# ubisoft/ubisoft-laforge-msmd

Measured on AMD Instinct MI355X. Metric: FLAME frames/sec on 4s@16kHz clips (whole job; MSMD.forward motion-coefficient frames), higher is better.
Workload: dtype bf16; 1 GPU; configs[1]: MSMD.forward, batch=32 x 4 s clips per GPU, wav2vec2-base encoder + 8-layer motion decoder, eval-mode, synthetic closed-form weights; batch_per_gpu=32, frames_per_clip=100, parallelism=dp1 (independent clips, no collective), launch=one hipGraph replay per step (the batch sits in the captured input buffers)

## Files before the change

include/msmd_hip.h:

```cpp
#ifndef MSMD_HIP_H
#define MSMD_HIP_H

#include <stdint.h>

#ifdef __cplusplus
extern "C" {
#endif

#define MSMD_F32 0
#define MSMD_BF16 1
#define MSMD_F16 2
#define MSMD_F16X2 3

#define MSMD_ACT_NONE 0
#define MSMD_ACT_GELU 1
#define MSMD_ACT_ELU 2

typedef void* msmd_stream_t;

int msmd_abi_version(void);
#define MSMD_GEMM_VARIANT(v) ((v) << 8)
#define MSMD_GEMM_WRITE_THROUGH (1 << 16)
#define MSMD_GEMM_PAIRED_STORES (1 << 17)
#define MSMD_GEMM_STAGGER (1 << 18)
// ... 21 lines not shown
                 long ldr, int act, int batch, long strideA, long strideW, long strideC, long strideBias, long strideR,
                 void* z_out, float p_drop, const unsigned long* rng_state, unsigned int site, msmd_stream_t stream);

int msmd_gemm_route(const void* A, const void* W, const float* bias, const void* residual, void* C, int M, int N, int K,
                    int in_dtype, int out_dtype, long lda, int rows_per_batch, long a_batch_stride, long ldw, long ldc,
                    long ldr, int act, int batch, long strideA, long strideW, long strideC, long strideBias, long strideR,
                    void* z_out, float p_drop, const unsigned long* rng_state, unsigned int site, msmd_stream_t stream);
int msmd_gemm_ln_route(const void* A, const void* W, const float* bias, const void* residual, void* C, int M, int N, int K,
                       int in_dtype, int out_dtype, long lda, long ldw, long ldc, long ldr, int act, const float* a_stats,
                       const float* w_colsum, const float* r_stats, const float* r_gamma, const float* r_beta,
                       float* stats_out, int slab_in, int slab_out, float eps, msmd_stream_t stream);
int msmd_gemm_ln_rows(const void* A, const void* W, const float* bias, const void* residual, void* C, int M, int N, int K,
                      int in_dtype, int out_dtype, long lda, long ldw, long ldc, long ldr, int act, const float* a_stats,
                      const float* w_colsum, const float* r_stats, const float* r_gamma, const float* r_beta,
                      float* stats_out, int slab_in, int slab_out, float eps, msmd_stream_t stream);

int msmd_gemm_actbwd(const void* A, const void* W, const void* Z, void* C, int M, int N, int K, int in_dtype, int out_dtype,
                     long lda, long ldw, int act, float p_drop, const unsigned long* rng_state, unsigned int site,
                     msmd_stream_t stream);

int msmd_gemm_batched2(const void* A, const void* W, void* C, int M, int N, int K, int in_dtype, int out_dtype,
                       long lda, long ldw, long ldc, int batch_outer, long strideA_o, long strideW_o, long strideC_o,
                       int batch_inner, long strideA_i, long strideW_i, long strideC_i, msmd_stream_t stream);

int msmd_gemm_tn(const void* A, const void* B, float* C, float* colsum, int M, int N, int K, long lda, long ldb,
                 long ldc, int batch, long strideA, long strideB, long strideC, int b_rows_per_window,
                 long b_window_stride, int accumulate, void* ws, long ws_bytes, msmd_stream_t stream);
long msmd_gemm_tn_workspace(int M, int N, int K, int batch);

int msmd_layernorm(const void* x, const void* residual, const float* gamma, const float* beta,
// ... 361 lines not shown
```

ubisoft-laforge-msmd_amd/csrc/gemm.hip:

```cpp
#include "gemm_tiles.h"
#include <atomic>
#include <utility>

struct GemmArgs {
  const void* A; const void* W; const float* bias; const void* R; void* C;
  int M, N, K;
  long lda; int rows_per_batch; long a_batch_stride; long ldw, ldc, ldr;
  int act; int vec_ok; float inv_rpb;
  long strideA, strideW, strideC, strideBias, strideR;
  int mt, nt;
  int batch_inner; long strideA2, strideW2, strideC2;
  void* Z; float p_drop; const unsigned long* rng; unsigned site;
  int xn;
  int flags;
  const float* a_stats = nullptr; int a_nt = 0; const float* w_colsum = nullptr;
  const float* r_stats = nullptr; int r_nt = 0; const float* r_gamma = nullptr; const float* r_beta = nullptr;
  float* stats_out = nullptr; float ln_eps = 1e-5f;
  int stagger_ticks = 0;
};

enum : int {
  GF_WRITE_THROUGH = 1, GF_PAIRED_STORES = 2, GF_STAGGER = 4,
  GF_ACT_BWD = 8,
  GF_ONE_TILE = 16, GF_NO_256 = 32,
// ... 905 lines not shown
        }
    }
    stage = ring_next<NSTAGE>(stage);
  }
#pragma unroll
  for (int i = 0; i < FN; ++i)
#pragma unroll
    for (int j = 0; j < FM; ++j)
#pragma unroll
      for (int e = 0; e < 4; ++e)
        acc0[i][j][e] = WS ? acc0[i][j][e] * MSMD_SPLIT_INV : fmaf(acc1[i][j][e], MSMD_SPLIT_INV, acc0[i][j][e]);
  if constexpr (sizeof(TO) == 4) gemm_epilogue<float, FM, FN, false, false, ACTK>(p, acc0, z, m0 + wm, n0 + wn, fr, fq);
  else gemm_epilogue_split<FM, FN, ACTK>(p, acc0, z, m0 + wm, n0 + wn, fr, fq);
}

template <typename TI, int EPIA, int SPLIT = 0>
__global__ __launch_bounds__(512) __attribute__((amdgpu_waves_per_eu(2, 2))) void gemm8_kernel(const GemmArgs p) {
  typedef typename std::conditional<(SPLIT & 3) == 2, float, TI>::type TO;
  constexpr bool WS = (SPLIT & 4) != 0;
  constexpr int EPI = epia_family(EPIA), ACTK = epia_act(EPIA);
  static_assert(SPLIT == 0 || (EPI == 1 && __is_same(TI, f16_t)), "split operands: fp16 planes, plain epilogue");
  constexpr int HALF = 128 * 128;
  constexpr int BUF = 4 * HALF;
  extern __shared__ __attribute__((aligned(16))) unsigned char smem[];

  const int pid = blockIdx.x, ntiles = p.mt * p.nt, nwg = gridDim.x;
  const int xcd = pid & 7;
  const int run0 = (xcd < (ntiles & 7) ? xcd * ((ntiles >> 3) + 1) : (ntiles & 7) * ((ntiles >> 3) + 1) + (xcd - (ntiles & 7)) * (ntiles >> 3));
  const int run_n = (ntiles >> 3) + (xcd < (ntiles & 7) ? 1 : 0);
  const int stride = (nwg >> 3) + (xcd < (nwg & 7) ? 1 : 0);
  int tl = pid >> 3;
  const bf16_t* __restrict__ A = (const bf16_t*)p.A;
  const bf16_t* __restrict__ W = (const bf16_t*)p.W;
  const int tid = threadIdx.x, lane = tid & 63;
  const int wid = __builtin_amdgcn_readfirstlane(tid >> 6);
  const int wr = wid >> 2, wc = wid & 3;

  unsigned src[4][2];
  int m0 = 0, n0 = 0;
  auto set_tile = [&](int t) {
    const int m_tile = (run0 + t) / p.nt, n_tile = (run0 + t) - m_tile * p.nt;
    m0 = m_tile * 256; n0 = n_tile * 256;
    int ln = lane;
    asm volatile("" : "+v"(ln));
#pragma unroll
    for (int i = 0; i < 2; ++i) {
      const int row = (i * 8 + wid) * 8 + (ln >> 3), phys = ln & 7;
      const int c = phys ^ ((row >> 1) & 7);
#pragma unroll
      for (int h = 0; h < 2; ++h) {
        src[h][i] = (unsigned)((a_row_offset(p, min(m0 + h * 128 + row, p.M - 1)) + c * 8) * 2);
        src[2 + h][i] = (unsigned)(((long)min(n0 + h * 128 + row, p.N - 1) * p.ldw + c * 8) * 2);
      }
    }
  };
  const unsigned dma_base = wid * 1024;
  auto stage = [&](int which, int kt, unsigned bufoff) {
// ... 105 lines not shown
        int ll = lane;
        asm volatile("" : "+v"(ll));
        const int m = min(m0 + ((ll >> 2) & 3) * 64 + wid * 8 + (ll & 3) * 2, p.M - 2);
#pragma unroll
        for (int q = 0; q < 4; ++q) {
          if (4 * q < ln_nt) {
            const int t = min(4 * q + (ll >> 4), ln_nt - 1);
            __builtin_amdgcn_global_load_lds((gbl_void_t*)(ln_stats + ((long)t * p.M + m) * 2),
                                             (lds_void_t*)(smem + (2 * BUF + wid * 4096 + q * 1024)), 16, 0, 0);
          }
        }
      }
    }
  };

  const int nk = p.K / (SPLIT ? 32 : 64);
  typedef typename Vec4T<TO>::type V4;
  const bool has_r = p.R != nullptr;
  const bool wt = p.flags & GF_WRITE_THROUGH;

  set_tile(tl);
  ln_request();
  stage(2, 0, 0); stage(0, 0, 0); stage(3, 0, 0); stage(1, 0, 0);
  stage(2, 1, BUF); stage(0, 1, BUF); stage(3, 1, BUF);
  asm volatile("s_waitcnt vmcnt(6)" ::: "memory");
  __builtin_amdgcn_s_barrier();

  while (true) {
    if (wr == 1) __builtin_amdgcn_s_barrier();
#pragma unroll
    for (int h = 0; h < 2; ++h)
#pragma unroll
      for (int g = 0; g < 2; ++g)
#pragma unroll
        for (int i = 0; i < 2; ++i)
#pragma unroll
          for (int j = 0; j < 4; ++j) acc[h][g][i][j] = f32x4{0.f, 0.f, 0.f, 0.f};
    unsigned cur = 0;
    auto ktile = [&](int t, auto MODE_) {
      constexpr int MODE = decltype(MODE_)::value;
      read_w(0, fw0);
      __builtin_amdgcn_sched_barrier(0);
      read_x(0);
      if (MODE <= 1) stage(1, t + 1, cur ^ BUF);
      asm volatile("s_waitcnt lgkmcnt(8)" ::: "memory");
      if constexpr (WS) scale_w(fw0, fs0);
      G8_BAR();
      quadrant(acc[0][0], fw0, fs0);
      G8_BAR();
      read_w(1, fw1);
      if (MODE == 0) stage(2, t + 2, cur);
      if constexpr (WS) {
        asm volatile("s_waitcnt lgkmcnt(0)" ::: "memory");
        scale_w(fw1, fs1);
      }
      G8_BAR();
      quadrant(acc[0][1], fw1, fs1);
      G8_BAR();
      read_x(1);
      if (MODE == 0) stage(0, t + 2, cur);
      G8_BAR();
      quadrant(acc[1][1], fw1, fs1);
      G8_BAR();
      if (MODE == 0) stage(3, t + 2, cur);
      if (MODE == 0) asm volatile("s_waitcnt vmcnt(6)" ::: "memory");
      if (MODE == 1) asm volatile("s_waitcnt vmcnt(0)" ::: "memory");
      G8_BAR();
      quadrant(acc[1][0], fw0, fs0);
      G8_BAR();
      cur ^= BUF; xa0 ^= BUF; xa1 ^= BUF; wa0 ^= BUF; wa1 ^= BUF;
    };
    for (int t = 0; t < nk - 2; ++t) ktile(t, std::integral_constant<int, 0>{});
    ktile(nk - 2, std::integral_constant<int, 1>{});
    ktile(nk - 1, std::integral_constant<int, 2>{});
    if (wr == 0) __builtin_amdgcn_s_barrier();
    if (nk & 1) { xa0 ^= BUF; xa1 ^= BUF; wa0 ^= BUF; wa1 ^= BUF; }

    const int em0 = m0, en0 = n0;
    int el = lane;
    asm volatile("" : "+v"(el));
    const int efr = el & 15, efq = el >> 4;
    const int ncol = en0 + el * 4;
    f32x4 cbias = f32x4{0.f, 0.f, 0.f, 0.f}, cx = f32x4{1.f, 1.f, 1.f, 1.f}, cy = f32x4{0.f, 0.f, 0.f, 0.f};
    if (p.bias) cbias = *(const f32x4*)(p.bias + ncol);
    if constexpr (EPI == 2) cx = *(const f32x4*)(p.w_colsum + ncol);
    if constexpr (EPI == 3) {
      if (p.r_stats) { cx = *(const f32x4*)(p.r_gamma + ncol); cy = *(const f32x4*)(p.r_beta + ncol); }
    }
    float mu_l = 0.f, rs_l = 1.f;
    if constexpr (EPI >= 2) {
      if (ln_stats) {
        const int r32 = el & 31;
        const unsigned base = 2 * BUF + wid * 4096 + (((r32 >> 3) * 4 + ((r32 & 7) >> 1)) << 4) + ((r32 & 1) << 3);
        float Sf[4], Qf[4];
#pragma unroll
        for (int f = 0; f < 4; ++f) {
          f32x2 w[4];
#pragma unroll
          for (int q = 0; q < 4; ++q) {
// ... 5 lines not shown
          Qf[f] = (w[0][1] + w[1][1]) + (w[2][1] + w[3][1]);
        }
        if (ln_nt > 16) {
          const f32x2* rp = (const f32x2*)ln_stats + min(em0 + (r32 >> 3) * 64 + wid * 8 + (r32 & 7), p.M - 1);
#pragma unroll
          for (int f = 0; f < 4; ++f)
            for (int t = 16 + f; t < ln_nt; t += 4) { const f32x2 w = rp[(long)t * p.M]; Sf[f] += w[0]; Qf[f] += w[1]; }
        }
        const float S = (Sf[0] + Sf[1]) + (Sf[2] + Sf[3]), Q = (Qf[0] + Qf[1]) + (Qf[2] + Qf[3]);
        const float inv_cols = 1.0f / (float)(EPI == 2 ? p.K : p.N);
        mu_l = S * inv_cols;
        rs_l = rsqrtf(fmaxf(Q * inv_cols - mu_l * mu_l, 0.f) + p.ln_eps);
        asm volatile("s_waitcnt lgkmcnt(0)" ::: "memory");
      }
    }
    tl += stride;
    const bool more = tl < run_n;
    if (more) {
      set_tile(tl);
      stage(2, 0, 0); stage(0, 0, 0); stage(3, 0, 0); stage(1, 0, 0);
      ln_request();
    }
    auto write_block = [&](const f32x4 (&q0)[2][4], const f32x4 (&q1)[2][4]) {
#pragma unroll
      for (int g = 0; g < 2; ++g)
#pragma unroll
        for (int i = 0; i < 2; ++i)
#pragma unroll
          for (int j = 0; j < 4; ++j) {
            const int row = j * 16 + efr, c = g * 32 + wc * 8 + i * 4 + efq;
            *(f32x4*)(smem + BUF + row * 1024 + ((c ^ efr) << 4)) = g == 0 ? q0[i][j] : q1[i][j];
          }
    };
    auto finish_block = [&](int ps) {
      if constexpr ((SPLIT & 3) == 2) {
        f32x4 rr[8];
        if (has_r) {
#pragma unroll
          for (int it = 0; it < 8; ++it) {
            const int m = min(em0 + ps * 64 + wid * 8 + it, p.M - 1);
            rr[it] = *(const f32x4*)((const float*)p.R + (long)m * p.ldr + ncol);
          }
        }
#pragma unroll
        for (int it = 0; it < 8; ++it) {
          const int row = wid * 8 + it, m = em0 + ps * 64 + row;
          const f32x4 a = *(const f32x4*)(smem + BUF + row * 1024 + ((el ^ (row & 15)) << 4));
          f32x4 o;
#pragma unroll
          for (int e = 0; e < 4; ++e) {
            o[e] = act_out_c<float, ACTK>(WS ? fmaf(a[e], MSMD_SPLIT_INV, cbias[e]) : a[e] + cbias[e], p.act);
            if (has_r) o[e] += rr[it][e];
          }
          if (m < p.M) {
            if (wt) store16_wt((float*)p.C + (long)m * p.ldc + ncol, __builtin_bit_cast(u32x4, o));
            else *(f32x4*)((float*)p.C + (long)m * p.ldc + ncol) = o;
          }
        }
      } else if constexpr ((SPLIT & 3) == 1) {
        const bool odd = el & 1;
        const long coff = 2L * en0 + ((el >> 3) << 6) + (((el >> 1) & 3) << 3) + (odd ? 32 : 0);
        auto swap1 = [](unsigned x) { return (unsigned)__builtin_amdgcn_mov_dpp((int)x, 0xB1, 0xF, 0xF, false); };
        u32x4 rr[8];
        if (has_r) {
#pragma unroll
          for (int it = 0; it < 8; ++it) {
            const int m = min(em0 + ps * 64 + wid * 8 + it, p.M - 1);
            rr[it] = *(const u32x4*)((const f16_t*)p.R + (long)m * 2 * p.ldr + coff);
          }
        }
#pragma unroll
        for (int it = 0; it < 8; ++it) {
          const int row = wid * 8 + it, m = em0 + ps * 64 + row;
          const f32x4 a = *(const f32x4*)(smem + BUF + row * 1024 + ((el ^ (row & 15)) << 4));
          float v[4];
#pragma unroll
          for (int e = 0; e < 4; ++e) v[e] = act_split<ACTK>(WS ? fmaf(a[e], MSMD_SPLIT_INV, cbias[e]) : a[e] + cbias[e], p.act);
          if (has_r) {
            const unsigned g0 = swap1(odd ? rr[it][0] : rr[it][2]), g1 = swap1(odd ? rr[it][1] : rr[it][3]);
            const f16x2 h01 = __builtin_bit_cast(f16x2, odd ? g0 : rr[it][0]), h23 = __builtin_bit_cast(f16x2, odd ? g1 : rr[it][1]);
            const f16x2 l01 = __builtin_bit_cast(f16x2, odd ? rr[it][2] : g0), l23 = __builtin_bit_cast(f16x2, odd ? rr[it][3] : g1);
            v[0] += unsplit_f16x2(h01[0], l01[0]); v[1] += unsplit_f16x2(h01[1], l01[1]);
            v[2] += unsplit_f16x2(h23[0], l23[0]); v[3] += unsplit_f16x2(h23[1], l23[1]);
          }
          f16_t h[4], l[4];
#pragma unroll
          for (int e = 0; e < 4; ++e) split_f16x2(v[e], h[e], l[e]);
          const unsigned hp0 = __builtin_bit_cast(unsigned, f16x2{h[0], h[1]}), hp1 = __builtin_bit_cast(unsigned, f16x2{h[2], h[3]});
          const unsigned lp0 = __builtin_bit_cast(unsigned, f16x2{l[0], l[1]}), lp1 = __builtin_bit_cast(unsigned, f16x2{l[2], l[3]});
          const unsigned g0 = swap1(odd ? hp0 : lp0), g1 = swap1(odd ? hp1 : lp1);
          const u32x4 o = odd ? u32x4{g0, g1, lp0, lp1} : u32x4{hp0, hp1, g0, g1};
          if (m < p.M) {
            if (wt) store16_wt((f16_t*)p.C + (long)m * 2 * p.ldc + coff, o);
            else *(u32x4*)((f16_t*)p.C + (long)m * 2 * p.ldc + coff) = o;
          }
        }
      } else {
      V4 rr[8];
      if (EPI != 2 && has_r) {
#pragma unroll
        for (int it = 0; it < 8; ++it) {
          const int m = min(em0 + ps * 64 + wid * 8 + it, p.M - 1);
          rr[it] = *(const V4*)((const TO*)p.R + (long)m * p.ldr + ncol);
        }
      }
#pragma unroll
      for (int it = 0; it < 8; ++it) {
        const int row = wid * 8 + it, m = em0 + ps * 64 + row;
        const f32x4 a = *(const f32x4*)(smem + BUF + row * 1024 + ((el ^ (row & 15)) << 4));
        float mu = 0.f, rs = 1.f;
        if constexpr (EPI >= 2) {
          mu = __int_as_float(__builtin_amdgcn_readlane(__float_as_int(mu_l), ps * 8 + it));
          rs = __int_as_float(__builtin_amdgcn_readlane(__float_as_int(rs_l), ps * 8 + it));
        }
        float v[4];
#pragma unroll
        for (int e = 0; e < 4; ++e) {
          float x = a[e];
          if constexpr (EPI == 2) x = rs * (x - mu * cx[e]);
          v[e] = act_out_c<TO, ACTK>(x + cbias[e], p.act);
          if constexpr (EPI == 3) v[e] += fmaf(((float)rr[it][e] - mu) * rs, cx[e], cy[e]);
          else if (has_r) v[e] += (float)rr[it][e];
        }
        const V4 o = pack4<TO>(v[0], v[1], v[2], v[3]);
        if (m < p.M) {
          if (wt) store8_wt((TO*)p.C + (long)m * p.ldc + ncol, __builtin_bit_cast(u32x2, o));
          else *(V4*)((TO*)p.C + (long)m * p.ldc + ncol) = o;
        }
        if constexpr (EPI == 3) {
          if (p.stats_out) {
            float S = 0.f, Q = 0.f;
#pragma unroll
            for (int e = 0; e < 4; ++e) { const float w = (float)o[e]; S += w; Q = fmaf(w, w, Q); }
#pragma unroll
            for (int d : {4, 8, 1, 2}) { S += __shfl_xor(S, d, 64); Q += __shfl_xor(Q, d, 64); }
            if ((el & 15) == 0 && m < p.M) *(f32x2*)(p.stats_out + ((long)((en0 >> 6) + (el >> 4)) * p.M + m) * 2) = f32x2{S, Q};
          }
        }
      }
      }
    };
    if (wr == 0) write_block(acc[0][0], acc[0][1]);
    G8_EBAR();
    finish_block(0);
    G8_EBAR();
    if (wr == 1) write_block(acc[0][0], acc[0][1]);
    G8_EBAR();
    finish_block(1);
    G8_EBAR();
    if (wr == 0) write_block(acc[1][0], acc[1][1]);
    G8_EBAR();
    finish_block(2);
    G8_EBAR();
    if (wr == 1) write_block(acc[1][0], acc[1][1]);
    G8_EBAR();
    finish_block(3);
    if (!more) break;
    G8_EBAR();
    set_tile(tl);
    stage(2, 1, BUF); stage(0, 1, BUF); stage(3, 1, BUF);
    asm volatile("s_waitcnt vmcnt(6)" ::: "memory");
    __builtin_amdgcn_s_barrier();
  }
#undef G8_BAR
#undef G8_EBAR
}

template <int... CODES, typename F>
static int dispatch_code(int code, F&& f) {
  int r = -1;
  (void)((code == CODES && ((r = f(std::integral_constant<int, CODES>{})), true)) || ...);
  return r;
}

template <auto KFN>
static int gemm_launch_kernel(dim3 grid, int threads, int lds, hipStream_t st, const GemmArgs& p) {
  if (lds > 0) {
    static std::atomic<unsigned long> allowed{0};
    int dev = 0;
    (void)hipGetDevice(&dev);
    const unsigned long bit = (unsigned)dev < 64 ? 1UL << dev : 0;
    if (!(allowed.load(std::memory_order_relaxed) & bit)) {
      (void)hipFuncSetAttribute((const void*)KFN, hipFuncAttributeMaxDynamicSharedMemorySize, lds);
      allowed.fetch_or(bit, std::memory_order_relaxed);
    }
  }
  hipLaunchKernelGGL(KFN, grid, dim3(threads), lds, st, p);
  MSMD_RETURN_LAST();
}

static int gemm2_xcd_grid(GemmArgs& p, int BM, int BN, long lda) {
  p.mt = (p.M + BM - 1) / BM; p.nt = (p.N + BN - 1) / BN;
  const double a_bytes = 2.0 * p.M * (double)(p.rows_per_batch < p.M ? lda : p.K), w_bytes = 2.0 * p.N * (double)p.K;
  double best = 1e30;
  int want_xn = 1;
  for (int xn = 1; xn <= 4; xn *= 2) {
    const double c = 0.7 * xn * a_bytes + (8.0 / xn) * w_bytes;
    if (c < best && p.nt >= xn) { best = c; want_xn = xn; }
  }
  p.xn = p.nt >= want_xn ? want_xn : 1;
  const int xm_n = 8 / p.xn;
  return ((p.mt + xm_n - 1) / xm_n) * ((p.nt + p.xn - 1) / p.xn) * 8;
// ... 433 lines not shown
  c.lda = lda; c.ldw = ldw; c.ldc = N; c.act = act & (0xffff | MSMD_GEMM_WRITE_THROUGH | MSMD_GEMM_PAIRED_STORES);
  c.z_out = const_cast<void*>(Z); c.p_drop = p_drop; c.rng = rng_state; c.site = site; c.internal_flags = GF_ACT_BWD;
  return gemm_run(gemm_plan, c, stream);
}

extern "C" int msmd_gemm_batched2(const void* A, const void* W, void* C, int M, int N, int K, int in_dtype, int out_dtype, long lda, long ldw,
                                  long ldc, int batch_outer, long strideA_o, long strideW_o, long strideC_o, int batch_inner, long strideA_i,
                                  long strideW_i, long strideC_i, msmd_stream_t stream) {
  GemmCall c;
  c.A = A; c.W = W; c.C = C; c.M = M; c.N = N; c.K = K; c.in_dtype = in_dtype; c.out_dtype = out_dtype;
  c.lda = lda; c.ldw = ldw; c.ldc = ldc; c.act = MSMD_ACT_NONE;
  c.batch = batch_outer; c.strideA = strideA_o; c.strideW = strideW_o; c.strideC = strideC_o;
  c.batch_inner = batch_inner; c.strideA2 = strideA_i; c.strideW2 = strideW_i; c.strideC2 = strideC_i;
  return gemm_run(gemm_plan, c, stream);
}
```

ubisoft-laforge-msmd_amd/ops.py:

```python
from __future__ import annotations

import ctypes
import functools
import os

import numpy as np
import torch
from torch.autograd.function import once_differentiable

from . import _lib

_HEADER = _lib.parse_constants()


def _h(*names):
    vals = tuple(_HEADER["MSMD_" + n] for n in names)
    return vals if len(vals) > 1 else vals[0]


F32, BF16, F16, F16X2 = _h("F32", "BF16", "F16", "F16X2")
SPLIT = "f16x2"


class Split:
# ... 382 lines not shown
    _lib.check(lib.msmd_gemm_tn(_p(a), _p(b), _p(out), _p(cs), M, N, K, lda, ldb, K, batch, strideA, strideB, N * K,
                                b_rows_per_window, b_window_stride, int(bool(accumulate)) | (int(splits) << 8), _p(ws), nws,
                                _stream()), "msmd_gemm_tn")
    return (out, cs) if (want_colsum or colsum_out is not None) else out


def conv1d_cl(x, w_packed, bias=None, *, kernel, stride, act=ACT_NONE, out_dtype=None):
    B, T, C = x.shape
    T_out = (T - kernel) // stride + 1
    out = empty((B, T_out, w_packed.shape[0]), x.device, out_dtype or x.dtype)
    gemm(x, w_packed, bias, None, act, out=out, M=B * T_out, K=kernel * C, lda=stride * C, rows_per_batch=T_out,
         a_batch_stride=T * C)
    return out


def layernorm(x, gamma, beta, residual=None, post_add=None, act=ACT_NONE, eps=1e-5, out_dtype=None, post_act=ACT_NONE,
              split=None):
    _need_cuda(x, gamma, beta)
    lib = _lib.load()
    cols = x.shape[-1]
    rows = x.numel() // cols
    if split:
        if x.dtype != torch.float32 or (residual is not None and residual.dtype != torch.float32):
            raise TypeError("layernorm(split=...) takes fp32 input")
        y = torch.empty(x.shape, device=x.device, dtype=torch.float32) if split == "both" else None
        ys = empty(tuple(x.shape), x.device, SPLIT)
        _lib.check(lib.msmd_layernorm_f16x2(_p(x), _p(residual), _p(gamma), _p(beta), _p(post_add), _p(y), _p(ys), rows,
                                            cols, eps, act | (post_act << 8), _stream()), "msmd_layernorm_f16x2")
        return (y, ys) if split == "both" else ys
    y = torch.empty(x.shape, device=x.device, dtype=out_dtype or x.dtype)
# ... 1367 lines not shown
```

ubisoft-laforge-msmd_amd/train_graph.py:

```python
from __future__ import annotations

import os
from types import SimpleNamespace

import numpy as np
import torch

from . import autograd as ag
from . import ops
from .utils.model_common import pad_audio_plan
from .utils.wav2vec2 import compute_mask_indices, compute_mask_indices_hf


USE_CONV3_FN = os.environ.get("MSMD_CONV3_FN", "1") != "0"


def _p(tree, name):
    return tree.get(name) if hasattr(tree, "get") else getattr(tree, name)


class PosConvFn(torch.autograd.Function):

    @staticmethod
    def forward(ctx, h, w, bias):
# ... 188 lines not shown
    if noise.graph_safe:
        coins = torch.rand((groups, 1, 1) if groups > 1 else (), device=h.device) < p
    else:
        rng = noise.host_rng if noise.host_rng is not None else np.random
        drawn = [rng.rand() < p for _ in range(groups)]
        if all(drawn) or not any(drawn):
            return all(drawn), None
        coins = torch.tensor(drawn, device=h.device).view(groups, 1, 1)
    return False, coins.repeat_interleave(h.shape[0] // groups, 0) if groups > 1 else coins


def audio_encoder_train(enc, audio, output_fps, frame_num, dtype, groups=1):
    c = enc.config
    with torch.no_grad():
        r, rep = pad_audio_plan(audio.shape[1])
        x = enc.feature_extractor_cl(audio, dtype, r, rep)
        T50 = x.shape[1]
        crop = min(round(frame_num * 50 / output_fps), T50)
        if not (crop == T50 and frame_num == T50):
            x = ops.interp_linear(x, frame_num, crop)
    g = lambda n: enc.get_parameter(n)
    noise = ag.TrainNoise
    h = ag.layer_norm(x, g("feature_projection.layer_norm.weight"), g("feature_projection.layer_norm.bias"))
    h = ag.linear_dropout(h, g("feature_projection.projection.weight"), g("feature_projection.projection.bias"),
                          c.feat_proj_dropout)
    if noise.active and c.apply_spec_augment and c.mask_time_prob > 0:
        m = noise.next_spec_mask()
        if m is not None and groups > 1 and m.shape[0] * groups == h.shape[0]:
            m = torch.cat([m] + [noise.next_spec_mask() for _ in range(groups - 1)], 0)
        if m is None:
            fn = compute_mask_indices_hf if enc.model_type == "hubert" else compute_mask_indices
# ... 405 lines not shown
```

ubisoft-laforge-msmd_amd/training_script.py:

```python
from __future__ import annotations

import contextlib
import os

import numpy as np
import torch

from . import autograd as ag
from . import dp, ops, synth
from . import train_graph as tg


def load_loss_weights(args, device=None):
    w = {"noise": 1.0, "vert": float(args.l_vert), "vel": float(args.l_vel), "smooth": float(args.l_smooth),
         "head_angle": float(args.l_head_angle), "head_vel": float(args.l_head_vel),
         "head_smooth": float(args.l_head_smooth), "head_trans": float(args.l_head_trans)}
    if not args.use_vertex_space:
        w["vel"] *= 4.5e-8
        w["smooth"] *= 4e-7
    legacy = args.dataset_type[:9] == "HDTF_TFHP" or args.dataset_type == "flame_mead_ravdess"
    if not legacy and args.use_vertex_space:
        w["vert"] *= 1e-7
        w["vel"] *= 1e-7
        w["smooth"] *= 2e-8
# ... 296 lines not shown
        eps = draws["eps"][i] if "eps" in draws else torch.randn_like(motion_in)
        ns, na = self._cfg_masks(draws, i, B)
        shape_in = torch.zeros_like(shape) if getattr(args, "do_ignore_shape", False) else shape
        return dict(style=style, end_idx=end_idx, audio_in=audio_in, motion_in=motion_in, indicator=indicator, ts=ts, eps=eps,
                    ns=ns, na=na, shape_in=shape_in)

    def _hand_off(self, batch, W0, audio_feat, dtype):
        model, n_prev = self.model, self.args.n_prev_motions
        if W0["end_idx"] is None:
            return W0["motion_in"][:, -n_prev:].detach(), audio_feat[:, -n_prev:].detach()
        audio = batch[0][0]
        with torch.no_grad():
            if ag.TrainNoise.active:
                prev_audio = tg.audio_feat_train(model, audio, model.n_motions, dtype).float()[:, -n_prev:]
            else:
                prev_audio = model.extract_audio_feature(audio)[:, -n_prev:]
        return batch[1][0][:, -n_prev:], prev_audio

    def _loss_terms(self, i, W, target, prev_motion, shape, mu, logvar, terms, lw):
        args = self.args
        prev = prev_motion if i == 1 else None
        if self.vertex_space:
            pairs = tg.loss_vert_train(args, i == 0, shape, W["motion_in"], target, prev, self.coef_stats, self.flame,
                                       W["end_idx"]).items()
        else:
            tup = tg.loss_no_vert_train(args, i == 0, W["motion_in"], target, prev, W["end_idx"],
                                        halve=False)
            pairs = zip(("noise", "vel", "smooth", "head_angle", "head_vel", "head_smooth", "head_trans"),
                        [(v, 0.5) for v in tup[:6]] + [(tup[6], 1.0)])
        for key, val in pairs:
            val, sc = val if isinstance(val, tuple) else (val, 1.0)
# ... 454 lines not shown
```

ubisoft-laforge-msmd_amd/utils/wav2vec2.py:

```python
from __future__ import annotations

from types import SimpleNamespace

import torch
import torch.nn as nn

from .. import ops, shapes, synth
from ..blocks import Rows, add, materialise, norm, project
from .model_common import ParamTree, pad_audio_plan

CONV_KERNEL = shapes.CONV_KERNEL
CONV_STRIDE = shapes.CONV_STRIDE


def compute_mask_indices(shape, mask_prob, mask_length, min_masks=0, rng=None):
    import numpy as np
    rng = np.random if rng is None else rng
    bsz, T = shape
    n_mask = max(min_masks, int(mask_prob * T / float(mask_length) + rng.rand()))
    spans = []
    for _ in range(bsz):
        lengths = np.full(n_mask, mask_length)
        if lengths.sum() == 0:
            lengths[0] = min(mask_length, T - 1)
# ... 92 lines not shown


def load_hf_state_dict(directory):
    import os
    st = os.path.join(directory, "model.safetensors")
    if os.path.isfile(st):
        from safetensors.torch import load_file
        return load_file(st, device="cpu")
    sd = torch.load(os.path.join(directory, "pytorch_model.bin"), map_location="cpu", weights_only=True)
    return sd.get("state_dict", sd) if isinstance(sd, dict) else sd


class Wav2Vec2Model(nn.Module):

    model_type = "wav2vec2"

    def __init__(self, config=None):
        super().__init__()
        cfg = dict(num_hidden_layers=12, hidden_size=768, intermediate_size=3072, num_attention_heads=12,
                   conv_dim=512, num_conv_pos_embeddings=128, num_conv_pos_embedding_groups=16,
                   layer_norm_eps=1e-5, output_attentions=False,
                   feat_extract_norm="group", conv_bias=False, do_stable_layer_norm=False,
                   hidden_dropout=0.1, attention_dropout=0.1, activation_dropout=0.1, feat_proj_dropout=0.1,
                   layerdrop=0.1, apply_spec_augment=True, mask_time_prob=0.05, mask_time_length=10,
                   mask_time_min_masks=2)
        if config is not None:
            cfg.update({k: v for k, v in (config if isinstance(config, dict) else vars(config)).items() if v is not None})
        self.config = SimpleNamespace(**cfg)
        c = self.config
        if isinstance(c.conv_dim, (tuple, list)):
# ... 137 lines not shown
                  and c.intermediate_size % 128 == 0 and sd["encoder.layer_norm.weight"].is_cuda)
        if P.fold:
            for n, L in enumerate(P.layers):
                p = f"encoder.layers.{n}."
                wqkv = torch.cat([sd[p + f"attention.{x}_proj.weight"] for x in ("q", "k", "v")], 0)
                w1 = sd[p + "feed_forward.intermediate_dense.weight"]
                if c.do_stable_layer_norm:
                    L.f_qkv = ops.fold_layernorm(wqkv, L.bqkv, *L.ln1, dtype)
                    L.f_w1 = ops.fold_layernorm(w1, L.b1, *L.ln2, dtype)
                else:
                    L.f_qkv = ops.fold_layernorm(wqkv, L.bqkv, *P.layers[n - 1].ln2, dtype) if n else None
                    L.f_w1 = ops.fold_layernorm(w1, L.b1, *L.ln1, dtype)
        self._packed, self._packed_dtype = P, (dtype, split)
        return P

    def feature_extractor_cl(self, audio, dtype, reflect_len=None, replicate_len=None):
        P = self.pack_fe(dtype)
        if reflect_len is None:
            reflect_len, replicate_len = 0, 0
        eps = self.config.layer_norm_eps
        if self.config.feat_extract_norm == "layer":
            x = ops.conv0_ln_gelu(audio.float().contiguous(), P.w0, P.conv_b[0], *P.conv_ln[0], reflect_len,
                                  replicate_len, dtype, eps)
            for i, w in enumerate(P.conv_w):
                z = ops.conv1d_cl(x, w, P.conv_b[i + 1], kernel=CONV_KERNEL[i + 1], stride=CONV_STRIDE[i + 1])
                x = ops.layernorm(z, *P.conv_ln[i + 1], post_act=ops.ACT_GELU, eps=eps)
            return x
        if P.split:
            x = ops.conv0_gn_gelu(audio.float().contiguous(), P.w0, P.gn_g, P.gn_b, reflect_len, replicate_len,
                                  ops.SPLIT, eps)
            for i, w in enumerate(P.conv_w):
                last = i == len(P.conv_w) - 1
                x = ops.conv1d_cl(x, w, P.conv_b[i + 1], kernel=CONV_KERNEL[i + 1], stride=CONV_STRIDE[i + 1],
                                  act=ops.ACT_GELU, out_dtype=torch.float32 if last else ops.SPLIT)
            return x
        x = ops.conv0_gn_gelu(audio.float().contiguous(), P.w0, P.gn_g, P.gn_b, reflect_len, replicate_len, dtype, eps)
        for i, w in enumerate(P.conv_w):
            x = ops.conv1d_cl(x, w, P.conv_b[i + 1], kernel=CONV_KERNEL[i + 1], stride=CONV_STRIDE[i + 1],
                              act=ops.ACT_GELU)
        return x

    def encode_features(self, x, dtype):
        P = self.pack(dtype)
        c = self.config
        B, T, _ = x.shape
        H, d, eps = c.num_attention_heads, c.hidden_size, c.layer_norm_eps
        scale = (d // H) ** -0.5
        pre = c.do_stable_layer_norm
        split = P.split and not pre
        fold = P.fold and ops.FOLD_LN
        h = ops.gemm(ops.layernorm(x, *P.fp_ln, eps=eps, split="only" if split else None), P.fp_w, P.fp_b)
        G, cg, kpos = c.num_conv_pos_embedding_groups, d // c.num_conv_pos_embedding_groups, c.num_conv_pos_embeddings
# ... 57 lines not shown
```

Baseline: 854,600 frames/s.

## Chain four wav2vec2 conv layers in one persistent GEMM kernel with dataflow tickets

Adds a persistent chained-GEMM kernel that runs conv layers 1-4 of the wav2vec2 feature extractor in a single launch. Workgroups claim tiles through an atomic ticket counter and spin-wait on per-row-block completion counters from the previous layer. Dependent layers can therefore overlap instead of draining and relaunching between layers. The cost is atomics, spin waits with a timeout, a workspace zeroing memset, and a risk of stalls or deadlock if scheduling goes wrong. It is on by default for the inference path and disabled in the training paths.

```diff
diff --git a/include/msmd_hip.h b/include/msmd_hip.h
--- a/include/msmd_hip.h
+++ b/include/msmd_hip.h
@@ -59,6 +59,17 @@
                       int in_dtype, int out_dtype, long lda, long ldw, long ldc, long ldr, int act, const float* a_stats,
                       const float* w_colsum, const float* r_stats, const float* r_gamma, const float* r_beta,
                       float* stats_out, int slab_in, int slab_out, float eps, msmd_stream_t stream);
+
+#define MSMD_CONV_CHAIN_RELEASE 1
+#define MSMD_CONV_CHAIN_ROW_BLOCK_TICKETS 2
+#define MSMD_CONV_CHAIN_TIMEOUT 1
+int msmd_conv_chain(const void* x, int B, int T0, int C, int N, int n_layers, const void* const* w, const float* const* bias,
+                    void* const* out, const int* kernel, const int* stride, int act, int dtype, void* workspace,
+                    long workspace_bytes, int max_workgroups, int flags, msmd_stream_t stream);
+long msmd_conv_chain_workspace(int B, int T0, int C, int N, int n_layers, const int* kernel, const int* stride);
+int msmd_conv_chain_plan(int B, int T0, int C, int N, int n_layers, const int* kernel, const int* stride, int flags, int ticket,
+                         int* out6);
+int msmd_conv_chain_status(const void* workspace);
 
 int msmd_gemm_actbwd(const void* A, const void* W, const void* Z, void* C, int M, int N, int K, int in_dtype, int out_dtype,
                      long lda, long ldw, int act, float p_drop, const unsigned long* rng_state, unsigned int site,
diff --git a/ubisoft-laforge-msmd_amd/csrc/gemm.hip b/ubisoft-laforge-msmd_amd/csrc/gemm.hip
--- a/ubisoft-laforge-msmd_amd/csrc/gemm.hip
+++ b/ubisoft-laforge-msmd_amd/csrc/gemm.hip
@@ -943,8 +943,49 @@
   else gemm_epilogue_split<FM, FN, ACTK>(p, acc0, z, m0 + wm, n0 + wn, fr, fq);
 }
 
-template <typename TI, int EPIA, int SPLIT = 0>
-__global__ __launch_bounds__(512) __attribute__((amdgpu_waves_per_eu(2, 2))) void gemm8_kernel(const GemmArgs p) {
+struct ChainProblem {
+  const void* A; const void* W; const float* bias; void* C;
+  long lda, a_batch_stride;
+  int M, rows_per_batch, K, mt;
+  int t_in, stride, taps;
+  int ticket0, cnt0;
+  float inv_rpb;
+};
+struct ChainTable {
+  ChainProblem pr[4];
+  unsigned* state;
+  int n, nt, per_block, total;
+  int release;
+};
+struct NoChain : ChainTable {};
+struct ChainTile { int l, rb, ct, nct, pb0, pb1; };
+constexpr int CHAIN_STATE_HEAD = 4;
+constexpr long CHAIN_WAIT_TICKS = 2000000;
+
+__host__ __device__ inline bool chain_decode(const ChainTable& t, int ticket, ChainTile& o) {
+  if (ticket < 0 || ticket >= t.total) return false;
+  int l = 0;
+  for (int i = 1; i < t.n; ++i)
+    if (ticket >= t.pr[i].ticket0) l = i;
+  const ChainProblem& q = t.pr[l];
+  const int local = ticket - q.ticket0;
+  o.l = l; o.pb0 = 0; o.pb1 = -1;
+  if (t.per_block) { o.rb = local; o.ct = 0; o.nct = t.nt; }
+  else { o.rb = local / t.nt; o.ct = local - o.rb * t.nt; o.nct = 1; }
+  if (l > 0) {
+    const int r0 = o.rb * 256, r1 = (r0 + 255 < q.M ? r0 + 255 : q.M - 1);
+    const int q0 = r0 / q.rows_per_batch, q1 = r1 / q.rows_per_batch;
+    const int first = q0 * q.t_in + (r0 - q0 * q.rows_per_batch) * q.stride;
+    const int last = q1 * q.t_in + (r1 - q1 * q.rows_per_batch) * q.stride + q.taps - 1;
+    o.pb0 = first >> 8; o.pb1 = last >> 8;
+  }
+  return true;
+}
+
+template <typename TI, int EPIA, int SPLIT, typename PA, typename CH>
+__device__ __forceinline__ void gemm8_body(PA& p, const CH& ch) {
+  constexpr bool CHAIN = !std::is_same_v<CH, NoChain>;
+  static_assert(!CHAIN || (SPLIT == 0 && epia_family(EPIA) == EPI_PLAIN), "the chained form: 16-bit operands, plain epilogue");
   typedef typename std::conditional<(SPLIT & 3) == 2, float, TI>::type TO;
   constexpr bool WS = (SPLIT & 4) != 0;
   constexpr int EPI = epia_family(EPIA), ACTK = epia_act(EPIA);
@@ -959,17 +1000,63 @@
   const int run_n = (ntiles >> 3) + (xcd < (ntiles & 7) ? 1 : 0);
   const int stride = (nwg >> 3) + (xcd < (nwg & 7) ? 1 : 0);
   int tl = pid >> 3;
-  const bf16_t* __restrict__ A = (const bf16_t*)p.A;
-  const bf16_t* __restrict__ W = (const bf16_t*)p.W;
+  const bf16_t* A = (const bf16_t*)p.A;
+  const bf16_t* W = (const bf16_t*)p.W;
   const int tid = threadIdx.x, lane = tid & 63;
   const int wid = __builtin_amdgcn_readfirstlane(tid >> 6);
   const int wr = wid >> 2, wc = wid & 3;
 
+  ChainTile cz{};
+  int c_left = 0;
+  volatile int* mbox = (volatile int*)(smem + 2 * BUF);
+  unsigned c_claim = 0, c_cnt = 0;
+  auto chain_problem = [&]() {
+    if constexpr (CHAIN) {
+      const ChainProblem& q = ch.pr[cz.l];
+      p.A = q.A; p.W = q.W; p.bias = q.bias; p.C = q.C; p.M = q.M; p.K = q.K; p.ldw = q.K;
+      p.lda = q.lda; p.a_batch_stride = q.a_batch_stride; p.rows_per_batch = q.rows_per_batch; p.inv_rpb = q.inv_rpb;
+      A = (const bf16_t*)q.A; W = (const bf16_t*)q.W;
+    }
+  };
+  auto chain_counters = [&](const ChainTile& z) -> unsigned {
+    unsigned c = ~0u;
+    if constexpr (CHAIN) {
+      if (z.l > 0) {
+        const unsigned* cnt = ch.state + CHAIN_STATE_HEAD + ch.pr[z.l - 1].cnt0;
+        c = (unsigned)ch.nt;
+        for (int b = z.pb0 + lane; b <= z.pb1; b += 64) {
+          const unsigned v = __hip_atomic_load(cnt + b, __ATOMIC_RELAXED, __HIP_MEMORY_SCOPE_AGENT);
+          c = v < c ? v : c;
+        }
+      }
+    }
+    return c;
+  };
+  auto chain_wait = [&](const ChainTile& z) -> bool {
+    if constexpr (CHAIN) {
+      if (z.l == 0) return true;
+      const long t0 = (long)__builtin_amdgcn_s_memrealtime();
+      while (!__all(chain_counters(z) >= (unsigned)ch.nt)) {
+        if ((long)__builtin_amdgcn_s_memrealtime() - t0 > CHAIN_WAIT_TICKS) {
+          if (lane == 0) __hip_atomic_store(ch.state + 1, (unsigned)MSMD_CONV_CHAIN_TIMEOUT, __ATOMIC_RELAXED, __HIP_MEMORY_SCOPE_AGENT);
+          return false;
+        }
+        __builtin_amdgcn_s_sleep(8);
+      }
+      __builtin_amdgcn_fence(__ATOMIC_ACQUIRE, "agent");
+      asm volatile("s_waitcnt vmcnt(0)" ::: "memory");
+    }
+    return true;
+  };
+
   unsigned src[4][2];
   int m0 = 0, n0 = 0;
   auto set_tile = [&](int t) {
-    const int m_tile = (run0 + t) / p.nt, n_tile = (run0 + t) - m_tile * p.nt;
-    m0 = m_tile * 256; n0 = n_tile * 256;
+    if constexpr (CHAIN) { m0 = cz.rb * 256; n0 = cz.ct * 256; }
+    else {
+      const int m_tile = (run0 + t) / p.nt, n_tile = (run0 + t) - m_tile * p.nt;
+      m0 = m_tile * 256; n0 = n_tile * 256;
+    }
     int ln = lane;
     asm volatile("" : "+v"(ln));
 #pragma unroll
@@ -1105,11 +1192,26 @@
     }
   };
 
-  const int nk = p.K / (SPLIT ? 32 : 64);
+  int nk = p.K / (SPLIT ? 32 : 64);
   typedef typename Vec4T<TO>::type V4;
   const bool has_r = p.R != nullptr;
   const bool wt = p.flags & GF_WRITE_THROUGH;
 
+  if constexpr (CHAIN) {
+    if (wid == 0) {
+      if (lane == 0) c_claim = __hip_atomic_fetch_add(ch.state, 1u, __ATOMIC_RELAXED, __HIP_MEMORY_SCOPE_AGENT);
+      const int tk = __builtin_amdgcn_readfirstlane((int)c_claim);
+      const bool ok = chain_decode(ch, tk, cz) && chain_wait(cz);
+      if (lane == 0) mbox[0] = ok ? tk : -1;
+    }
+    __syncthreads();
+    const int tk = __builtin_amdgcn_readfirstlane(mbox[0]);
+    if (tk < 0) return;
+    chain_decode(ch, tk, cz);
+    c_left = cz.nct - 1;
+    chain_problem();
+    nk = p.K / 64;
+  }
   set_tile(tl);
   ln_request();
   stage(2, 0, 0); stage(0, 0, 0); stage(3, 0, 0); stage(1, 0, 0);
@@ -1130,6 +1232,9 @@
     unsigned cur = 0;
     auto ktile = [&](int t, auto MODE_) {
       constexpr int MODE = decltype(MODE_)::value;
+      if constexpr (CHAIN && MODE == 1) {
+        if (wid == 0 && c_left == 0 && lane == 0) c_claim = __hip_atomic_fetch_add(ch.state, 1u, __ATOMIC_RELAXED, __HIP_MEMORY_SCOPE_AGENT);
+      }
       read_w(0, fw0);
       __builtin_amdgcn_sched_barrier(0);
       read_x(0);
@@ -1156,6 +1261,15 @@
       if (MODE == 0) stage(3, t + 2, cur);
       if (MODE == 0) asm volatile("s_waitcnt vmcnt(6)" ::: "memory");
       if (MODE == 1) asm volatile("s_waitcnt vmcnt(0)" ::: "memory");
+      if constexpr (CHAIN && MODE == 1) {
+        if (wid == 0 && c_left == 0) {
+          const int tk = __builtin_amdgcn_readfirstlane((int)c_claim);
+          ChainTile nz;
+          const bool ok = chain_decode(ch, tk, nz);
+          c_cnt = ok ? chain_counters(nz) : ~0u;
+          if (lane == 0) mbox[0] = ok ? tk : -1;
+        }
+      }
       G8_BAR();
       quadrant(acc[1][0], fw0, fs0);
       G8_BAR();
@@ -1164,16 +1278,37 @@
     for (int t = 0; t < nk - 2; ++t) ktile(t, std::integral_constant<int, 0>{});
     ktile(nk - 2, std::integral_constant<int, 1>{});
     ktile(nk - 1, std::integral_constant<int, 2>{});
+    if constexpr (CHAIN) {
+      if (wid == 0 && c_left == 0) {
+        const bool ready = __all(c_cnt >= (unsigned)ch.nt);
+        if (ready && __builtin_amdgcn_readfirstlane((int)c_cnt) != -1) {
+          __builtin_amdgcn_fence(__ATOMIC_ACQUIRE, "agent");
+          asm volatile("s_waitcnt vmcnt(0)" ::: "memory");
+        }
+        if (lane == 0) mbox[1] = ready;
+        asm volatile("s_waitcnt lgkmcnt(0)" ::: "memory");
+      }
+    }
     if (wr == 0) __builtin_amdgcn_s_barrier();
     if (nk & 1) { xa0 ^= BUF; xa1 ^= BUF; wa0 ^= BUF; wa1 ^= BUF; }
 
     const int em0 = m0, en0 = n0;
+    const int eM = p.M;
+    void* const eC = p.C;
+    const float* const ebias = p.bias;
+    bool e_pub = false, ewt = wt;
+    unsigned* e_cnt = nullptr;
+    if constexpr (CHAIN) {
+      e_pub = cz.l + 1 < ch.n;
+      ewt = e_pub ? !ch.release : true;
+      e_cnt = ch.state + CHAIN_STATE_HEAD + ch.pr[cz.l].cnt0 + cz.rb;
+    }
     int el = lane;
     asm volatile("" : "+v"(el));
     const int efr = el & 15, efq = el >> 4;
     const int ncol = en0 + el * 4;
     f32x4 cbias = f32x4{0.f, 0.f, 0.f, 0.f}, cx = f32x4{1.f, 1.f, 1.f, 1.f}, cy = f32x4{0.f, 0.f, 0.f, 0.f};
-    if (p.bias) cbias = *(const f32x4*)(p.bias + ncol);
+    if (ebias) cbias = *(const f32x4*)(ebias + ncol);
     if constexpr (EPI == 2) cx = *(const f32x4*)(p.w_colsum + ncol);
     if constexpr (EPI == 3) {
       if (p.r_stats) { cx = *(const f32x4*)(p.r_gamma + ncol); cy = *(const f32x4*)(p.r_beta + ncol); }
@@ -1209,11 +1344,28 @@
         asm volatile("s_waitcnt lgkmcnt(0)" ::: "memory");
       }
     }
-    tl += stride;
-    const bool more = tl < run_n;
+    bool more, ready = true;
+    if constexpr (CHAIN) {
+      if (c_left > 0) { --c_left; ++cz.ct; more = true; }
+      else {
+        const int tk = __builtin_amdgcn_readfirstlane(mbox[0]);
+        ready = __builtin_amdgcn_readfirstlane(mbox[1]) != 0;
+        more = tk >= 0;
+        if (more) {
+          chain_decode(ch, tk, cz);
+          c_left = cz.nct - 1;
+          chain_problem();
+          nk = p.K / 64;
+        }
+      }
+    } else {
+      tl += stride;
+      more = tl < run_n;
+    }
     if (more) {
       set_tile(tl);
-      stage(2, 0, 0); stage(0, 0, 0); stage(3, 0, 0); stage(1, 0, 0);
+      stage(2, 0, 0); if (ready) stage(0, 0, 0);
+      stage(3, 0, 0); if (ready) stage(1, 0, 0);
       ln_request();
     }
     auto write_block = [&](const f32x4 (&q0)[2][4], const f32x4 (&q1)[2][4]) {
@@ -1233,7 +1385,7 @@
         if (has_r) {
 #pragma unroll
           for (int it = 0; it < 8; ++it) {
-            const int m = min(em0 + ps * 64 + wid * 8 + it, p.M - 1);
+            const int m = min(em0 + ps * 64 + wid * 8 + it, eM - 1);
             rr[it] = *(const f32x4*)((const float*)p.R + (long)m * p.ldr + ncol);
           }
         }
@@ -1247,9 +1399,9 @@
             o[e] = act_out_c<float, ACTK>(WS ? fmaf(a[e], MSMD_SPLIT_INV, cbias[e]) : a[e] + cbias[e], p.act);
             if (has_r) o[e] += rr[it][e];
           }
-          if (m < p.M) {
-            if (wt) store16_wt((float*)p.C + (long)m * p.ldc + ncol, __builtin_bit_cast(u32x4, o));
-            else *(f32x4*)((float*)p.C + (long)m * p.ldc + ncol) = o;
+          if (m < eM) {
+            if (ewt) store16_wt((float*)eC + (long)m * p.ldc + ncol, __builtin_bit_cast(u32x4, o));
+            else *(f32x4*)((float*)eC + (long)m * p.ldc + ncol) = o;
           }
         }
       } else if constexpr ((SPLIT & 3) == 1) {
@@ -1260,7 +1412,7 @@
         if (has_r) {
 #pragma unroll
           for (int it = 0; it < 8; ++it) {
-            const int m = min(em0 + ps * 64 + wid * 8 + it, p.M - 1);
+            const int m = min(em0 + ps * 64 + wid * 8 + it, eM - 1);
             rr[it] = *(const u32x4*)((const f16_t*)p.R + (long)m * 2 * p.ldr + coff);
           }
         }
@@ -1285,9 +1437,9 @@
           const unsigned lp0 = __builtin_bit_cast(unsigned, f16x2{l[0], l[1]}), lp1 = __builtin_bit_cast(unsigned, f16x2{l[2], l[3]});
           const unsigned g0 = swap1(odd ? hp0 : lp0), g1 = swap1(odd ? hp1 : lp1);
           const u32x4 o = odd ? u32x4{g0, g1, lp0, lp1} : u32x4{hp0, hp1, g0, g1};
-          if (m < p.M) {
-            if (wt) store16_wt((f16_t*)p.C + (long)m * 2 * p.ldc + coff, o);
-            else *(u32x4*)((f16_t*)p.C + (long)m * 2 * p.ldc + coff) = o;
+          if (m < eM) {
+            if (ewt) store16_wt((f16_t*)eC + (long)m * 2 * p.ldc + coff, o);
+            else *(u32x4*)((f16_t*)eC + (long)m * 2 * p.ldc + coff) = o;
           }
         }
       } else {
@@ -1295,7 +1447,7 @@
       if (EPI != 2 && has_r) {
 #pragma unroll
         for (int it = 0; it < 8; ++it) {
-          const int m = min(em0 + ps * 64 + wid * 8 + it, p.M - 1);
+          const int m = min(em0 + ps * 64 + wid * 8 + it, eM - 1);
           rr[it] = *(const V4*)((const TO*)p.R + (long)m * p.ldr + ncol);
         }
       }
@@ -1318,9 +1470,9 @@
           else if (has_r) v[e] += (float)rr[it][e];
         }
         const V4 o = pack4<TO>(v[0], v[1], v[2], v[3]);
-        if (m < p.M) {
-          if (wt) store8_wt((TO*)p.C + (long)m * p.ldc + ncol, __builtin_bit_cast(u32x2, o));
-          else *(V4*)((TO*)p.C + (long)m * p.ldc + ncol) = o;
+        if (m < eM) {
+          if (ewt) store8_wt((TO*)eC + (long)m * p.ldc + ncol, __builtin_bit_cast(u32x2, o));
+          else *(V4*)((TO*)eC + (long)m * p.ldc + ncol) = o;
         }
         if constexpr (EPI == 3) {
           if (p.stats_out) {
@@ -1350,8 +1502,37 @@
     if (wr == 1) write_block(acc[1][0], acc[1][1]);
     G8_EBAR();
     finish_block(3);
-    if (!more) break;
-    G8_EBAR();
+    if constexpr (CHAIN) {
+      if (e_pub) {
+        asm volatile("s_waitcnt vmcnt(0)" ::: "memory");
+        G8_EBAR();
+        if (tid == 0) {
+          if (ch.release) {
+            __builtin_amdgcn_fence(__ATOMIC_RELEASE, "agent");
+            asm volatile("s_waitcnt vmcnt(0)" ::: "memory");
+          }
+          __hip_atomic_fetch_add(e_cnt, 1u, __ATOMIC_RELAXED, __HIP_MEMORY_SCOPE_AGENT);
+        }
+      }
+      if (!more) break;
+      if (!e_pub) G8_EBAR();
+      if (!ready) {
+        if (wid == 0) {
+          const bool ok = chain_wait(cz);
+          if (lane == 0) mbox[2] = ok;
+        }
+        __syncthreads();
+        if (!__builtin_amdgcn_readfirstlane(mbox[2])) {
+          asm volatile("s_waitcnt vmcnt(0)" ::: "memory");
+          break;
+        }
+        set_tile(tl);
+        stage(0, 0, 0); stage(1, 0, 0);
+      }
+    } else {
+      if (!more) break;
+      G8_EBAR();
+    }
     set_tile(tl);
     stage(2, 1, BUF); stage(0, 1, BUF); stage(3, 1, BUF);
     asm volatile("s_waitcnt vmcnt(6)" ::: "memory");
@@ -1359,6 +1540,16 @@
   }
 #undef G8_BAR
 #undef G8_EBAR
+}
+
+template <typename TI, int EPIA, int SPLIT = 0>
+__global__ __launch_bounds__(512) __attribute__((amdgpu_waves_per_eu(2, 2))) void gemm8_kernel(const GemmArgs p) {
+  gemm8_body<TI, EPIA, SPLIT>(p, NoChain{});
+}
+template <typename TI, int EPIA>
+__global__ __launch_bounds__(512) __attribute__((amdgpu_waves_per_eu(2, 2))) void gemm8_chain_kernel(const GemmArgs p0, const ChainTable ch) {
+  GemmArgs p = p0;
+  gemm8_body<TI, EPIA, 0>(p, ch);
 }
 
 template <int... CODES, typename F>
@@ -1368,8 +1559,8 @@
   return r;
 }
 
-template <auto KFN>
-static int gemm_launch_kernel(dim3 grid, int threads, int lds, hipStream_t st, const GemmArgs& p) {
+template <auto KFN, typename... ARGS>
+static int gemm_launch_kernel(dim3 grid, int threads, int lds, hipStream_t st, const ARGS&... p) {
   if (lds > 0) {
     static std::atomic<unsigned long> allowed{0};
     int dev = 0;
@@ -1380,7 +1571,7 @@
       allowed.fetch_or(bit, std::memory_order_relaxed);
     }
   }
-  hipLaunchKernelGGL(KFN, grid, dim3(threads), lds, st, p);
+  hipLaunchKernelGGL(KFN, grid, dim3(threads), lds, st, p...);
   MSMD_RETURN_LAST();
 }
 
@@ -1844,3 +2035,84 @@
   c.batch_inner = batch_inner; c.strideA2 = strideA_i; c.strideW2 = strideW_i; c.strideC2 = strideC_i;
   return gemm_run(gemm_plan, c, stream);
 }
+
+static bool conv_chain_table(ChainTable& t, int B, int T0, int C, int N, int n, const int* kernel, const int* stride, int flags) {
+  if (B <= 0 || T0 <= 0 || C <= 0 || N <= 0 || n < 2 || n > 4 || !kernel || !stride || (N % 256)) return false;
+  t = ChainTable{};
+  t.n = n; t.nt = N / 256;
+  t.per_block = (flags & MSMD_CONV_CHAIN_ROW_BLOCK_TICKETS) != 0;
+  t.release = (flags & MSMD_CONV_CHAIN_RELEASE) != 0;
+  long t_in = T0, c_in = C;
+  int tickets = 0, counters = 0;
+  for (int l = 0; l < n; ++l) {
+    ChainProblem& q = t.pr[l];
+    if (kernel[l] <= 0 || stride[l] <= 0 || t_in < kernel[l]) return false;
+    const long t_out = (t_in - kernel[l]) / stride[l] + 1, M = (long)B * t_out, K = kernel[l] * c_in;
+    if ((K % 64) || K < 128 || M >= (1L << 24)) return false;
+    q.M = (int)M; q.K = (int)K; q.rows_per_batch = (int)t_out; q.inv_rpb = 1.0f / (float)t_out;
+    q.lda = stride[l] * c_in; q.a_batch_stride = t_in * c_in;
+    q.t_in = (int)t_in; q.stride = stride[l]; q.taps = kernel[l];
+    q.mt = (int)((M + 255) / 256);
+    q.ticket0 = tickets; q.cnt0 = counters;
+    tickets += t.per_block ? q.mt : q.mt * t.nt;
+    counters += q.mt;
+    if (((long)(B - 1) * q.a_batch_stride + (t_out - 1) * q.lda + K) * 2 >= (1L << 32) || (long)N * K * 2 >= (1L << 32)) return false;
+    t_in = t_out; c_in = N;
+  }
+  t.total = tickets;
+  return true;
+}
+static long conv_chain_state_bytes(const ChainTable& t) {
+  const long words = CHAIN_STATE_HEAD + t.pr[t.n - 1].cnt0 + t.pr[t.n - 1].mt;
+  return (words * 4 + 15) / 16 * 16;
+}
+
+extern "C" long msmd_conv_chain_workspace(int B, int T0, int C, int N, int n_layers, const int* kernel, const int* stride) {
+  ChainTable t;
+  return conv_chain_table(t, B, T0, C, N, n_layers, kernel, stride, 0) ? conv_chain_state_bytes(t) : 0;
+}
+
+extern "C" int msmd_conv_chain_plan(int B, int T0, int C, int N, int n_layers, const int* kernel, const int* stride, int flags, int ticket,
+                                    int* out6) {
+  ChainTable t;
+  if (!out6 || !conv_chain_table(t, B, T0, C, N, n_layers, kernel, stride, flags)) return -1;
+  ChainTile z;
+  if (!chain_decode(t, ticket, z)) return t.total;
+  out6[0] = z.l; out6[1] = z.rb; out6[2] = z.ct; out6[3] = z.nct; out6[4] = z.pb0; out6[5] = z.pb1;
+  return 0;
+}
+
+extern "C" int msmd_conv_chain(const void* x, int B, int T0, int C, int N, int n_layers, const void* const* w, const float* const* bias,
+                               void* const* out, const int* kernel, const int* stride, int act, int dtype, void* workspace,
+                               long workspace_bytes, int max_workgroups, int flags, msmd_stream_t stream) {
+  ChainTable t;
+  if ((dtype != MSMD_BF16 && dtype != MSMD_F16) || (act != MSMD_ACT_NONE && act != MSMD_ACT_GELU) || !x || !w || !bias || !out || !workspace) return 1;
+  if (!conv_chain_table(t, B, T0, C, N, n_layers, kernel, stride, flags)) return 1;
+  const long state_bytes = conv_chain_state_bytes(t);
+  if (workspace_bytes < state_bytes || ((uintptr_t)workspace & 15) || max_workgroups < 0) return 1;
+  for (int l = 0; l < n_layers; ++l) {
+    ChainProblem& q = t.pr[l];
+    q.A = l ? out[l - 1] : x; q.W = w[l]; q.bias = bias[l]; q.C = out[l];
+    if (!q.W || !q.C || ((uintptr_t)q.A & 15) || ((uintptr_t)q.W & 15) || ((uintptr_t)q.bias & 15) || ((uintptr_t)q.C & 15)) return 1;
+  }
+  t.state = (unsigned*)workspace;
+  GemmArgs p{};
+  p.N = N; p.ldc = N; p.act = act; p.vec_ok = 1; p.batch_inner = 1; p.xn = 1; p.nt = t.nt;
+  p.A = t.pr[0].A; p.W = t.pr[0].W; p.C = t.pr[0].C; p.M = t.pr[0].M; p.K = t.pr[0].K;
+  const int cap = gemm8_workgroup_cap();
+  int grid = t.total < cap ? t.total : cap;
+  if (max_workgroups > 0 && max_workgroups < grid) grid = max_workgroups;
+  hipStream_t st = (hipStream_t)stream;
+  if (const hipError_t e = msmd_zero_async(workspace, (size_t)state_bytes, st); e != hipSuccess) return (int)e;
+  constexpr int LDS = GEMM8_RING + 16;
+  const int code = epia(EPI_PLAIN, act);
+  if (dtype == MSMD_BF16)
+    return dispatch_code<11, 21>(code, [&](auto c) { return gemm_launch_kernel<gemm8_chain_kernel<bf16_t, decltype(c)::value>>(dim3(grid), 512, LDS, st, p, t); });
+  return dispatch_code<11, 21>(code, [&](auto c) { return gemm_launch_kernel<gemm8_chain_kernel<f16_t, decltype(c)::value>>(dim3(grid), 512, LDS, st, p, t); });
+}
+
+extern "C" int msmd_conv_chain_status(const void* workspace) {
+  unsigned s = 0;
+  if (!workspace || hipMemcpy(&s, (const unsigned*)workspace + 1, sizeof(s), hipMemcpyDeviceToHost) != hipSuccess) return -1;
+  return (int)s;
+}
diff --git a/ubisoft-laforge-msmd_amd/ops.py b/ubisoft-laforge-msmd_amd/ops.py
--- a/ubisoft-laforge-msmd_amd/ops.py
+++ b/ubisoft-laforge-msmd_amd/ops.py
@@ -420,6 +420,59 @@
     return out
 
 
+CONV_CHAIN_RELEASE, CONV_CHAIN_ROW_BLOCK_TICKETS = _h("CONV_CHAIN_RELEASE", "CONV_CHAIN_ROW_BLOCK_TICKETS")
+CONV_CHAIN_FLAGS = 0
+
+
+def _int_array(vals):
+    return (ctypes.c_int * len(vals))(*[int(v) for v in vals])
+
+
+def conv_chain_plan(B, T0, C, N, kernels, strides, flags, ticket):
+    out = (ctypes.c_int * 6)()
+    r = _lib.load().msmd_conv_chain_plan(B, T0, C, N, len(kernels), _int_array(kernels), _int_array(strides), flags, ticket, out)
+    return None if r < 0 else (tuple(out) if r == 0 else r)
+
+
+def conv_chain_status(workspace):
+    return _lib.load().msmd_conv_chain_status(_p(workspace))
+
+
+def conv_chain(x, ws_packed, biases, *, kernels, strides, act=ACT_NONE, flags=None, max_workgroups=0, outs=None, workspace=None):
+    _need_cuda(x, *ws_packed, *biases)
+    lib = _lib.load()
+    B, T0, C = x.shape
+    n, N = len(ws_packed), ws_packed[0].shape[0]
+    if x.dtype not in (torch.bfloat16, torch.float16) or not x.is_contiguous() or any(w.dtype != x.dtype or not w.is_contiguous() for w in ws_packed):
+        return None
+    ks, ss = _int_array(kernels), _int_array(strides)
+    nbytes = lib.msmd_conv_chain_workspace(B, T0, C, N, n, ks, ss)
+    if nbytes <= 0:
+        return None
+    if outs is None:
+        outs, T = [], T0
+        for k, s in zip(kernels, strides):
+            T = (T - k) // s + 1
+            outs.append(torch.empty((B, T, N), device=x.device, dtype=x.dtype))
+    if workspace is None:
+        workspace = torch.empty(nbytes, device=x.device, dtype=torch.uint8)
+    Ms = [o.shape[0] * o.shape[1] for o in outs]
+    ptrs = lambda ts: (ctypes.c_void_p * n)(*[_p(t) for t in ts])
+    flags = CONV_CHAIN_FLAGS if flags is None else flags
+    Ks = [k * (C if l == 0 else N) for l, k in enumerate(kernels)]
+    if len(set(Ks)) == 1:
+        trace = _trace_begin(sum(Ms), N, Ks[0], 1, _dt(x))
+    else:
+        if GEMM_FLOPS is not None:
+            GEMM_FLOPS[0] += 2.0 * N * (sum(m * k for m, k in zip(Ms, Ks)) - sum(Ms[1:]) * Ks[1])
+        trace = _trace_begin(sum(Ms[1:]), N, Ks[1], 1, _dt(x))
+    r = lib.msmd_conv_chain(_p(x), B, T0, C, N, n, ptrs(ws_packed), ptrs(biases), ptrs(outs), ks, ss, act, _dt(x), _p(workspace),
+                            workspace.numel(), max_workgroups, flags, _stream())
+    _lib.check(r, "msmd_conv_chain")
+    _trace_end(trace, lambda: 80, ())
+    return outs
+
+
 def layernorm(x, gamma, beta, residual=None, post_add=None, act=ACT_NONE, eps=1e-5, out_dtype=None, post_act=ACT_NONE,
               split=None):
     _need_cuda(x, gamma, beta)
diff --git a/ubisoft-laforge-msmd_amd/train_graph.py b/ubisoft-laforge-msmd_amd/train_graph.py
--- a/ubisoft-laforge-msmd_amd/train_graph.py
+++ b/ubisoft-laforge-msmd_amd/train_graph.py
@@ -226,7 +226,7 @@
     c = enc.config
     with torch.no_grad():
         r, rep = pad_audio_plan(audio.shape[1])
-        x = enc.feature_extractor_cl(audio, dtype, r, rep)
+        x = enc.feature_extractor_cl(audio, dtype, r, rep, chain=False)
         T50 = x.shape[1]
         crop = min(round(frame_num * 50 / output_fps), T50)
         if not (crop == T50 and frame_num == T50):
diff --git a/ubisoft-laforge-msmd_amd/training_script.py b/ubisoft-laforge-msmd_amd/training_script.py
--- a/ubisoft-laforge-msmd_amd/training_script.py
+++ b/ubisoft-laforge-msmd_amd/training_script.py
@@ -334,7 +334,12 @@
             if ag.TrainNoise.active:
                 prev_audio = tg.audio_feat_train(model, audio, model.n_motions, dtype).float()[:, -n_prev:]
             else:
-                prev_audio = model.extract_audio_feature(audio)[:, -n_prev:]
+                enc = model.audio_encoder
+                chain, enc.conv_chain = enc.conv_chain, False
+                try:
+                    prev_audio = model.extract_audio_feature(audio)[:, -n_prev:]
+                finally:
+                    enc.conv_chain = chain
         return batch[1][0][:, -n_prev:], prev_audio
 
     def _loss_terms(self, i, W, target, prev_motion, shape, mu, logvar, terms, lw):
diff --git a/ubisoft-laforge-msmd_amd/utils/wav2vec2.py b/ubisoft-laforge-msmd_amd/utils/wav2vec2.py
--- a/ubisoft-laforge-msmd_amd/utils/wav2vec2.py
+++ b/ubisoft-laforge-msmd_amd/utils/wav2vec2.py
@@ -130,6 +130,7 @@
 class Wav2Vec2Model(nn.Module):
 
     model_type = "wav2vec2"
+    conv_chain = True
 
     def __init__(self, config=None):
         super().__init__()
@@ -297,7 +298,7 @@
         self._packed, self._packed_dtype = P, (dtype, split)
         return P
 
-    def feature_extractor_cl(self, audio, dtype, reflect_len=None, replicate_len=None):
+    def feature_extractor_cl(self, audio, dtype, reflect_len=None, replicate_len=None, chain=True):
         P = self.pack_fe(dtype)
         if reflect_len is None:
             reflect_len, replicate_len = 0, 0
@@ -318,7 +319,15 @@
                                   act=ops.ACT_GELU, out_dtype=torch.float32 if last else ops.SPLIT)
             return x
         x = ops.conv0_gn_gelu(audio.float().contiguous(), P.w0, P.gn_g, P.gn_b, reflect_len, replicate_len, dtype, eps)
+        first = 0
+        if self.conv_chain and chain and len(P.conv_w) >= 4:
+            outs = ops.conv_chain(x, P.conv_w[:4], P.conv_b[1:5], kernels=CONV_KERNEL[1:5], strides=CONV_STRIDE[1:5],
+                                  act=ops.ACT_GELU)
+            if outs is not None:
+                x, first = outs[-1], 4
         for i, w in enumerate(P.conv_w):
+            if i < first:
+                continue
             x = ops.conv1d_cl(x, w, P.conv_b[i + 1], kernel=CONV_KERNEL[i + 1], stride=CONV_STRIDE[i + 1],
                               act=ops.ACT_GELU)
         return x
```

Result: faster. 865,300 frames/s, median of 6 (+1.2%).
